# alessioGalatolo/GAN-2D-to-3D

Hardware: AMD Instinct MI355X
Metric: GAN2Shape step iters/sec, faces 128×128 b=8, 1/2/4/8 MI355X (higher is better)
Workload: dtype f32; 1 GPU; face128_n8; image_size=128, gan_size=128, n_proj_samples=8, mfma_operands=f32, prior=ellipsoid, step_mix=7:7:6 (step1:step2:step3, main.py:148 stage 0), images_per_rank=1

## Files before the change

### gan-2d-to-3d_amd/build.py

```python
import os
import subprocess
import sys

HERE = os.path.dirname(os.path.abspath(__file__))
CSRC = os.path.join(HERE, "csrc")
LIBDIR = os.path.join(HERE, "lib")
LIB = os.path.join(LIBDIR, "libg2s.so")
ARCH = "gfx950"

SOURCES = {
    "api.hip": [],
    "raster.hip": ["-ffp-contract=off"],
    "raster_rgb.hip": ["-ffp-contract=off"],
    "sweep.hip": ["-ffp-contract=off"],
    "face_light.hip": ["-ffp-contract=off"],
    "mapping.hip": ["-ffp-contract=off"],
    "fused_bias_act.hip": [],
    "upfirdn2d.hip": [],
    "modconv.hip": [],
    "modconv_f16.hip": [],
    "thinconv.hip": [],
    "winograd.hip": ["-fno-slp-vectorize"],
    "winograd4.hip": ["-fno-slp-vectorize"],
    "split_reduce.hip": [],
    "rowops.hip": [],
    "projector.hip": [],
    "synth_batch.hip": [],
    "lpips.hip": [],
    "pool.hip": [],
    "losses.hip": [],
    "geometry.hip": ["-ffp-contract=off"],
    "grid_sample.hip": ["-ffp-contract=off"],
    "priors.hip": ["-ffp-contract=off"],
    "metrics.hip": ["-ffp-contract=off"],
    "parsing.hip": [],
    "groupnorm.hip": [],
    "conv_wgrad.hip": [],
    "adam.hip": [],
    "probe.hip": [],
}
COMMON = ["--offload-arch=" + ARCH, "-O3", "-fPIC", "-std=c++17", "-Wall", "-Wno-unused-function",
          "-mllvm", "-instcombine-max-copied-from-constant-users=100000"]


def _newer(src, dst, deps):
    if not os.path.exists(dst):
        return True
    t = os.path.getmtime(dst)
    return any(os.path.getmtime(d) > t for d in [src] + deps)


def build(force=False, verbose=False):
    hipcc = os.environ.get("HIPCC", "/opt/rocm/bin/hipcc")
    os.makedirs(LIBDIR, exist_ok=True)
    headers = [os.path.join(CSRC, f) for f in os.listdir(CSRC) if f.endswith((".h", ".inc"))]
    headers.append(os.path.join(HERE, "..", "include", "g2s.h"))
    objs, jobs = [], []
    for name, extra in SOURCES.items():
        src = os.path.join(CSRC, name)
        if not os.path.exists(src):
            continue
# ... 26 lines not shown
```

### gan-2d-to-3d_amd/lib.py

```python
import ctypes as C
import os

import torch

_HERE = os.path.dirname(os.path.abspath(__file__))
LIB_PATH = os.path.join(_HERE, "lib", "libg2s.so")

G2S_F32, G2S_F16 = 0, 1
CONV_PLAIN, CONV_UP2, CONV_DOWN2 = 0, 1, 2

_lib = None

_p, _i, _f, _sz, _i64, _d = C.c_void_p, C.c_int, C.c_float, C.c_size_t, C.c_int64, C.c_double
SIGNATURES = {
    "g2s_abi_version": (_i, []),
    "g2s_last_error": (C.c_char_p, []),
    "g2s_clamp": (_i, [_p, _p, _p, _i64, _f, _f, _i, _p]),
    "g2s_avg_pyramid": (_i, [_p, _p, _i, _i64, _i, _i, _p]),
    "g2s_res_split_fwd": (_i, [_p, _p, _p, _i64, _i, _i, _p]),
    "g2s_res_split_bwd": (_i, [_p, _p, _p, _p, _i64, _i, _i, _p]),
    "g2s_depth_head_fwd": (_i, [_p, _p, _p, _i64, _i, _f, _f, _i, _f, _p]),
    "g2s_depth_head_bwd": (_i, [_p, _p, _p, _p, _p, _i64, _i, _f, _f, _i, _f, _i, _p]),
    "g2s_grid_sample_fwd": (_i, [_p, _p, _p, _i, _i, _i, _i, _i, _i, _i, _f, _f, _p]),
    "g2s_grid_sample_bwd_workspace_bytes": (_sz, [_i, _i, _i, _i]),
# ... 36 lines not shown
    "g2s_upfirdn2d_nba_ps": (_i, [_p, _p, _p] + [_i] * 12 + [_p, _p, _p, _f, _f, _p]),
    "g2s_synth_bwd_rows_ps": (_i, [_p] * 13 + [_i, _i, _i, _f, _f, _p]),
    "g2s_channel_sum": (_i, [_p, _p, _i, _i, _i, _p]),
    "g2s_noise_grad": (_i, [_p, _p, _p, _i, _i, _i, _p]),
    "g2s_noise_regularize_workspace_bytes": (_sz, [_p, _i, _i]),
    "g2s_noise_regularize": (_i, [_p, _p, _p, _i, _i, _p, _p, _sz, _p]),
    "g2s_noise_normalize_workspace_bytes": (_sz, [_p, _i, _i]),
    "g2s_noise_normalize": (_i, [_p, _p, _i, _i, _p, _sz, _p]),
    "g2s_demod_fwd_multi": (_i, [_p, _p, _p, _p, _p, _i, _i, _f, _p]),
    "g2s_demod_bwd_multi": (_i, [_p, _p, _p, _p, _p, _p, _p, _i, _i, _p]),
    "g2s_modconv_f16": (_i, [_p, _p, _p, _p, _p, _p, _i, _i, _i, _i, _i, _i, _i, _i, _i, _f, _f, _p]),
    "g2s_modconv_tune": (_i, [_i, _i]),
    "g2s_mfma_probe": (_i, [_p, _i, _i, _i, _p]),
    "g2s_mfma_lds_probe": (_i, [_p, _i, _i, _i, _i, _p]),
    "g2s_wino_weights_floats": (_sz, [_i, _i]),
    "g2s_wino4_weights_floats": (_sz, [_i, _i]),
    "g2s_wino4_weights": (_i, [_p, _p, _i, _i, _i, _p]),
    "g2s_wino4_supported": (_i, [_i] * 5),
    "g2s_conv3x3_wino4": (_i, [_p] * 8 + [_i] * 6 + [_f, _f, _i, _p, _i64, _p]),
    "g2s_wino_weights": (_i, [_p, _p, _i, _i, _i, _p]),
    "g2s_conv3x3_wino": (_i, [_p] * 8 + [_i] * 6 + [_f, _f, _i, _p, _i64, _p]),
    "g2s_conv2d": (_i, [_p, _p, _p, _p] + [_i] * 12 + [_i, _f, _f, _i, _i, _p]),
    "g2s_conv2d_wgrad": (_i, [_p, _p, _p] + [_i] * 10 + [_i, _i, _p]),
    "g2s_conv2d_bwd": (_i, [_p, _p, _p] + [_i] * 13 + [_p, _p, _p] + [_i] * 8 + [_p]),
    "g2s_adam_chunk": (_i64, []),
    "g2s_adam_step": (_i, [_p, _p, _p, _i, _i, _f, _f, _f, _f, _f, _p]),
    "g2s_rows_dot_scale": (_i, [_p, _p, _p, _p, _p, _p, _i, _i, _p]),
    "g2s_demod_fwd": (_i, [_p, _p, _p, _i, _i, _i, _f, _p]),
    "g2s_demod_bwd": (_i, [_p, _p, _p, _p, _p, _i, _i, _i, _p]),
    "g2s_demod_bwd_add": (_i, [_p, _p, _p, _p, _p, _p, _i, _i, _i, _p]),
    "g2s_lpips_layer_fwd": (_i, [_p, _p, _p, _p, _i, _i, _i, _p]),
    "g2s_lpips_layer_bwd": (_i, [_p, _p, _p, _p, _p, _i, _i, _i, _p]),
    "g2s_lpips_layer_bwd_ex": (_i, [_p, _p, _p, _p, _p, _i, _p, _i, _i, _i, _p]),
    "g2s_weighted_l1_fwd": (_i, [_p, _p, _p, _p, _i, _i, _i, _p]),
    "g2s_weighted_l1_bwd": (_i, [_p, _p, _p, _p, _p, _i, _i, _i, _p]),
    "g2s_weighted_l1_fwd2": (_i, [_p, _p, _p, _p, _i, _i, _i, _p]),
    "g2s_weighted_l1_bwd3": (_i, [_p] * 7 + [_f, _p, _p, _f, _f, _p, _i, _i, _i, _p]),
    "g2s_weighted_l1_bwd2": (_i, [_p, _p, _p, _p, _p, _p, _p, _i, _i, _i, _p]),
    "g2s_view_transform_fwd": (_i, [_p, _f, _f, _f, _p, _p, _i, _p]),
    "g2s_view_transform_bwd": (_i, [_p, _f, _f, _f, _p, _p, _p, _i, _p]),
    "g2s_warp_verts_fwd": (_i, [_p, _p, _p, _p, _f, _p, _i, _i, _p]),
    "g2s_warp_verts_bwd": (_i, [_p, _p, _p, _p, _f, _p, _p, _i, _i, _i, _p]),
    "g2s_inv_warp_grid_fwd": (_i, [_p, _p, _p, _p, _p, _f, _p, _i, _i, _i, _p]),
    "g2s_inv_warp_grid_bwd": (_i, [_p, _p, _p, _p, _p, _f, _p, _p, _p, _i, _i, _i, _i, _p]),
    "g2s_normal_fwd": (_i, [_p, _p, _p, _i, _i, _i, _p]),
    "g2s_normal_bwd": (_i, [_p, _p, _p, _p, _i, _i, _i, _p]),
    "g2s_shading_fwd": (_i, [_p, _p, _p, _p, _p, _i, _i, _i, _i, _p]),
    "g2s_shading_bwd": (_i, [_p, _p, _p, _p, _p, _p, _p, _p, _i, _i, _i, _i, _i, _p]),
    "g2s_smooth_loss_fwd": (_i, [_p, _p, _i, _i, _i, _i, _p]),
    "g2s_smooth_loss_bwd": (_i, [_p, _p, _p, _i, _i, _i, _p]),
    "g2s_groupnorm_workspace_floats": (_sz, [_i, _i, _i, _i]),
    "g2s_groupnorm_act_fwd": (_i, [_p, _p, _p, _p, _p, _p, _p, _i, _i, _i, _i, _f, _i, _f, _p]),
    "g2s_groupnorm_act_bwd": (_i, [_p, _p, _p, _p, _p, _p, _p, _p, _p, _p, _i, _i, _i, _i, _i, _f, _p]),
    "g2s_prior_map": (_i, [_p, _i, _i, _i, _d, _d, _p, _p]),
    "g2s_prior_smooth_workspace_bytes": (_sz, [_i, _i, _i, _i]),
    "g2s_prior_smooth": (_i, [_p, _i, _i, _i, _i, _d, _d, _p, _p, _sz, _p]),
    "g2s_prior_ellipsoid_workspace_bytes": (_sz, [_i]),
    "g2s_prior_ellipsoid": (_i, [_p, _i, _i, _d, _d, _d, _d, _p, _p, _sz, _p]),
    "g2s_conv_stem7": (_i, [_p, _p, _p, _p, _i, _i, _i, _i, _i, _p]),
    "g2s_maxpool3x3s2": (_i, [_p, _p, _i, _i, _i, _p]),
    "g2s_adaptive_avgpool": (_i, [_p, _p, _i, _i, _i, _i, _i, _p]),
    "g2s_resize_bilinear": (_i, [_p, _p, _i, _i, _i, _i, _i, _i, _p]),
    "g2s_gate_add_act": (_i, [_p, _p, _p, _p, _p, _i, _i, _i, _i, _i, _p]),
    "g2s_parse_head_workspace_bytes": (_sz, [_i]),
    "g2s_parse_head": (_i, [_p, _i, _i, _i, _i, _i, _i, _i, _i, C.c_uint32, _p, _p, _p, _p, _sz, _p]),
    "g2s_depth_metrics_workspace_bytes": (_sz, [_i, _i, _i]),
# ... 64 lines not shown
```

### gan-2d-to-3d_amd/lpips.py

```python
import torch
import torch.nn as nn
from torch.autograd import Function
from torch.autograd.function import once_differentiable

from . import lib as _lib
from . import zeropool

_VGG_SLICES = [
    [(0, 3, 64), (2, 64, 64)],
    [(5, 64, 128), (7, 128, 128)],
    [(10, 128, 256), (12, 256, 256), (14, 256, 256)],
    [(17, 256, 512), (19, 512, 512), (21, 512, 512)],
    [(24, 512, 512), (26, 512, 512), (28, 512, 512)],
]
_POOL_BEFORE = [None, 4, 9, 16, 23]


def normalize_tensor(in_feat, eps=1e-10):
    norm_factor = torch.sqrt(torch.sum(in_feat ** 2, dim=1, keepdim=True))
    return in_feat / (norm_factor + eps)


class _LpipsLayer(Function):

# ... 23 lines not shown

class _MaxPool2x2(Function):

    @staticmethod
    def forward(ctx, x):
        x = x.contiguous()
        B, C_, H, W = x.shape
        y = torch.empty((B, C_, H // 2, W // 2), dtype=torch.float32, device=x.device)
        _lib.check(_lib.load().g2s_maxpool2x2_fwd(_lib.ptr(x), _lib.ptr(y), B * C_, H, W, _lib.stream()))
        ctx.save_for_backward(x)
        return y

    @staticmethod
    def backward(ctx, gy):
        (x,) = ctx.saved_tensors
        B, C_, H, W = x.shape
        gx = torch.empty_like(x)
        _lib.check(_lib.load().g2s_maxpool2x2_bwd(_lib.ptr(x), _lib.ptr(gy.contiguous()), _lib.ptr(gx), B * C_, H, W,
                                                  _lib.stream()))
        return gx


def _pool_ok(mod):
    return (mod.kernel_size in (2, (2, 2)) and mod.stride in (2, (2, 2)) and mod.padding in (0, (0, 0))
            and not mod.ceil_mode and mod.dilation in (1, (1, 1)))


class _VggLpips(Function):

    SPLIT_FORWARD = False

    @staticmethod
    def forward(ctx, pred, target, net):
        from .modconv import conv_bias_act_raw
        N = pred.shape[0]
        sl = net.scaling_layer
        x = (torch.cat([pred, target], 0) - sl.shift) / sl.scale
        L = _lib.load()
        acc = zeropool.zeros(N, pred.device)
        saved = []
        for si in range(5):
            entry = {"pool_in": None, "convs": []}
            for mod in getattr(net.net, f"slice{si + 1}"):
                if isinstance(mod, nn.MaxPool2d):
                    entry["pool_in"] = x
                    B, C_, H, W = x.shape
                    y = torch.empty((B, C_, H // 2, W // 2), dtype=torch.float32, device=x.device)
                    _lib.check(L.g2s_maxpool2x2_fwd(_lib.ptr(x), _lib.ptr(y), B * C_, H, W, _lib.stream()))
                    x = y
                elif isinstance(mod, nn.Conv2d):
                    if _VggLpips.SPLIT_FORWARD:
                        x = torch.cat([conv_bias_act_raw(x[:N], mod.weight, mod.bias),
                                       conv_bias_act_raw(x[N:], mod.weight, mod.bias)], 0)
                    else:
                        x = conv_bias_act_raw(x, mod.weight, mod.bias)
                    entry["convs"].append((mod.weight, x))
            wv = getattr(net, f"lin{si}").model[-1].weight.reshape(-1).contiguous()
            C_, HW = x.shape[1], x.shape[2] * x.shape[3]
            _lib.check(L.g2s_lpips_layer_fwd(_lib.ptr(x[:N]), _lib.ptr(x[N:]), _lib.ptr(wv), _lib.ptr(acc),
                                             N, C_, HW, _lib.stream()))
            entry["lin"] = wv
            saved.append(entry)
        ctx.saved, ctx.N, ctx.scale = saved, N, sl.scale
        return acc.view(-1, 1, 1, 1)

    @staticmethod
    @once_differentiable
    def backward(ctx, gout):
        from .modconv import PLAIN, modconv_raw, relu_gate
        L = _lib.load()
        N = ctx.N
        gout = gout.contiguous().view(-1)
        g = None
        for si in range(4, -1, -1):
            e = ctx.saved[si]
            y = e["convs"][-1][1]
            C_, HW = y.shape[1], y.shape[2] * y.shape[3]
            gn = torch.empty((N,) + tuple(y.shape[1:]), dtype=torch.float32, device=y.device)
            _lib.check(L.g2s_lpips_layer_bwd_ex(_lib.ptr(y[:N]), _lib.ptr(y[N:]), _lib.ptr(e["lin"]), _lib.ptr(gout),
                                                _lib.ptr(g), 1, _lib.ptr(gn), N, C_, HW, _lib.stream()))
            g = gn
            convs = e["convs"]
            for ci in range(len(convs) - 1, -1, -1):
                w, yc = convs[ci]
                if ci != len(convs) - 1:
                    g = relu_gate(g, yc[:N])
                g = modconv_raw(g, w, None, None, PLAIN, 1)
            if e["pool_in"] is not None:
                xin = e["pool_in"]
                B2, C2, H, W = xin.shape
                gx = torch.empty((N, C2, H, W), dtype=torch.float32, device=xin.device)
                _lib.check(L.g2s_maxpool2x2_bwd(_lib.ptr(xin[:N]), _lib.ptr(g.contiguous()), _lib.ptr(gx), N * C2, H, W,
                                                _lib.stream()))
                g = gx
        return g / ctx.scale, None, None


def max_pool_2x2(mod, x):
    if (x.is_cuda and x.dtype == torch.float32 and x.dim() == 4 and x.shape[2] % 2 == 0 and x.shape[3] % 8 == 0
            and mod.kernel_size in (2, (2, 2)) and mod.stride in (2, (2, 2)) and mod.padding in (0, (0, 0))
            and not mod.ceil_mode and mod.dilation in (1, (1, 1))):
        return _MaxPool2x2.apply(x)
    return mod(x)


class VGG16Features(nn.Module):

    def __init__(self):
        super().__init__()
        for si, convs in enumerate(_VGG_SLICES):
            seq = nn.Sequential()
            if _POOL_BEFORE[si] is not None:
                seq.add_module(str(_POOL_BEFORE[si]), nn.MaxPool2d(kernel_size=2, stride=2))
            for idx, cin, cout in convs:
                seq.add_module(str(idx), nn.Conv2d(cin, cout, kernel_size=3, padding=1))
                seq.add_module(str(idx + 1), nn.ReLU(inplace=True))
            setattr(self, f"slice{si + 1}", seq)
        for p in self.parameters():
            p.requires_grad = False

    def forward(self, x):
        fused = x.is_cuda and x.dtype == torch.float32 and not any(p.requires_grad for p in self.parameters())
        outs = []
        for si in range(5):
            if fused:
                from .modconv import conv_bias_relu
                for mod in getattr(self, f"slice{si + 1}"):
                    if isinstance(mod, nn.Conv2d):
# ... 8 lines not shown

class ScalingLayer(nn.Module):
    def __init__(self):
        super().__init__()
        self.register_buffer('shift', torch.Tensor([-.030, -.088, -.188])[None, :, None, None])
        self.register_buffer('scale', torch.Tensor([.458, .448, .450])[None, :, None, None])

    def forward(self, inp):
        return (inp - self.shift) / self.scale


class NetLinLayer(nn.Module):
    def __init__(self, chn_in, chn_out=1, use_dropout=True):
        super().__init__()
        layers = [nn.Dropout()] if use_dropout else []
        layers += [nn.Conv2d(chn_in, chn_out, 1, stride=1, padding=0, bias=False)]
        self.model = nn.Sequential(*layers)


class PNetLin(nn.Module):

    ONE_NODE = True

    def __init__(self):
        super().__init__()
        self.scaling_layer = ScalingLayer()
        self.chns = [64, 128, 256, 512, 512]
        self.net = VGG16Features()
        for i, c in enumerate(self.chns):
            setattr(self, f"lin{i}", NetLinLayer(c))
        for p in self.parameters():
            p.requires_grad = False

    def features(self, x):
        return [normalize_tensor(f) for f in self.net(self.scaling_layer(x))]

    def forward(self, in0, in1):
        fused = in0.is_cuda and not in0.requires_grad and not any(
            getattr(self, f"lin{k}").model[-1].weight.requires_grad for k in range(5))
        if (fused and self.ONE_NODE and in0.dtype == torch.float32 and in0.shape == in1.shape
                and in0.shape[2] % 16 == 0 and in0.shape[3] % 64 == 0
                and not any(p.requires_grad for p in self.net.parameters())
                and all(_pool_ok(m) for s_ in range(1, 6) for m in getattr(self.net, f"slice{s_}")
                        if isinstance(m, nn.MaxPool2d))):
            return _VggLpips.apply(in1.contiguous(), in0.contiguous(), self)
        if not fused:
            f0, f1 = self.features(in0), self.features(in1)
            val = 0
            for k in range(5):
                diff = (f0[k] - f1[k]) ** 2
                val = val + getattr(self, f"lin{k}").model(diff).mean([2, 3], keepdim=True)
            return val
        with torch.no_grad():
            ft = self.net(self.scaling_layer(in0))
        fp = self.net(self.scaling_layer(in1))
        acc = torch.zeros(in1.shape[0], dtype=torch.float32, device=in1.device)
        for k in range(5):
            acc = _LpipsLayer.apply(fp[k], ft[k], getattr(self, f"lin{k}").model[-1].weight, acc)
        return acc.view(-1, 1, 1, 1)


class PerceptualLoss(nn.Module):

    def __init__(self, model='net-lin', net='vgg', use_gpu=True, gpu_ids=None,
                 lin_weights_path=None, vgg_weights_path=None):
        super().__init__()
        if model != 'net-lin' or net != 'vgg':
            raise NotImplementedError("only model='net-lin', net='vgg' (GAN2Shape/model.py:79)")
        self.net = PNetLin()
        self.pretrained = False
        if lin_weights_path is not None:
            self.load_lin_weights(lin_weights_path)
        if vgg_weights_path is not None:
            self.load_vgg_features(vgg_weights_path)
            self.pretrained = lin_weights_path is not None
        self.net.eval()

    def load_lin_weights(self, path):
        sd = path if isinstance(path, dict) else torch.load(path, map_location="cpu", weights_only=True)
        missing = self.net.load_state_dict(sd, strict=False)
        assert not [k for k in missing.unexpected_keys if k.startswith("lin")], missing

    def load_vgg_features(self, path):
        sd = path if isinstance(path, dict) else torch.load(path, map_location="cpu", weights_only=True)
        sd = {k.replace("features.", ""): v for k, v in sd.items() if "classifier" not in k}
        own = {}
        for si, convs in enumerate(_VGG_SLICES):
            for idx, _, _ in convs:
                for suffix in ("weight", "bias"):
                    own[f"slice{si + 1}.{idx}.{suffix}"] = sd[f"{idx}.{suffix}"]
        self.net.net.load_state_dict(own)

    def forward(self, pred, target, normalize=False):
        if normalize:
            target = 2 * target - 1
            pred = 2 * pred - 1
        return self.net(target, pred)
```

### gan-2d-to-3d_amd/model.py

```python
import datetime
import logging
import math
import os
from glob import glob

import torch
import torch.nn as nn
import torch.nn.functional as F
from torch.distributions.multivariate_normal import MultivariateNormal

from . import networks, utils, zeropool
from .op import grid_sample
from .losses import DiscriminatorLoss, PhotometricLoss, SmoothLoss
from .lpips import PerceptualLoss
from .renderer import Renderer
from .stylegan2 import Discriminator, Generator


_WSUM_CONST = {}


def weighted_total(terms):
    flat = [t.reshape(-1) for _, t in terms]
    per_elem = [tuple(float(v) for v in w) if isinstance(w, (tuple, list)) else (float(w) / f.numel(),) * f.numel()
                for (w, _), f in zip(terms, flat)]
    assert all(len(pe) == f.numel() for pe, f in zip(per_elem, flat))
    key = (tuple(per_elem), flat[0].device)
    wv = _WSUM_CONST.get(key)
    if wv is None:
        if flat[0].is_cuda and torch.cuda.is_current_stream_capturing():
            raise RuntimeError("weighted_total: first use of this weight vector under graph capture; run the step eagerly once")
        if len(_WSUM_CONST) > 64:
            _WSUM_CONST.clear()
        wv = _WSUM_CONST[key] = torch.tensor([v for pe in per_elem for v in pe], dtype=torch.float32).to(flat[0].device)
    return torch.dot(torch.cat(flat), wv)


class GAN2Shape(nn.Module):
    NETS = ['lighting', 'viewpoint', 'depth', 'albedo', 'offset_encoder']

    def __init__(self, config, debug=False, device="cuda"):
        super().__init__()
        self.device = torch.device(device)
        self.z_dim = config.get('z_dim')
        self.debug = debug
        self.generator = Generator(config.get('gan_size'), self.z_dim, 8,
                                   channel_multiplier=config.get('channel_multiplier'))
# ... 105 lines not shown
        if clamp_border:
            if self._depth_border is None or self._depth_border.shape[-2:] != (h, w):
                border = torch.zeros(1, h, w - 4, device=depth.device)
                self._depth_border = F.pad(border, (2, 2), mode='constant', value=1.02)
            depth = depth * (1 - self._depth_border) + self._depth_border * self.border_depth
        return depth

    def get_lighting_directions(self, lighting):
        lighting_a = lighting[:, :1] / 2 + 0.5
        lighting_b = lighting[:, 1:2] / 2 + 0.5
        lighting_d = torch.cat([lighting[:, 2:], lighting.new_ones(lighting.size(0), 1)], 1)
        lighting_d = lighting_d / ((lighting_d ** 2).sum(1, keepdim=True)) ** 0.5
        return lighting_a, lighting_b, lighting_d

    def get_shading(self, normal, lighting_a, lighting_b, lighting_d, albedo):
        diffuse_shading = (normal * lighting_d.view(-1, 1, 1, 3)).sum(3).clamp(min=0).unsqueeze(1)
        shading = lighting_a.view(-1, 1, 1, 1) + lighting_b.view(-1, 1, 1, 1) * diffuse_shading
        texture = (albedo / 2 + 0.5) * shading * 2 - 1
        return diffuse_shading, texture

    def _shade(self, normal, lighting, albedo):
        if lighting.is_cuda and self.renderer.fused:
            from .fused_geometry import shading
            diffuse_shading, texture = shading(normal, lighting, albedo)
            ab = lighting[:, :2] / 2 + 0.5
            return ab[:, :1], ab[:, 1:2], diffuse_shading, texture
        lighting_a, lighting_b, lighting_d = self.get_lighting_directions(lighting)
        diffuse_shading, texture = self.get_shading(normal, lighting_a, lighting_b, lighting_d, albedo)
        return lighting_a, lighting_b, diffuse_shading, texture

    @staticmethod
    def _head(x, n):
        return x if x.shape[0] == n else x[:n]

    def _no_grad_if(self, cond):
        return torch.no_grad() if cond else torch.enable_grad()

    def _fork(self, jobs):
        if len(jobs) < 2 or not self.parallel_nets or self.device.type != 'cuda':
            return [job() for job in jobs]
        main = torch.cuda.current_stream(self.device)
        while len(self._side_streams) < len(jobs) - 1:
            self._side_streams.append(torch.cuda.Stream(self.device))
        outs = [None] * len(jobs)
        for i, (job, side) in enumerate(zip(jobs[1:], self._side_streams), 1):
            side.wait_stream(main)
            with torch.cuda.stream(side):
                outs[i] = job()
        outs[0] = jobs[0]()
        for out, side in zip(outs[1:], self._side_streams):
            main.wait_stream(side)
            for t in (out if isinstance(out, (tuple, list)) else (out,)):
                t.record_stream(main)
        return outs

    def forward_step1(self, images, latents, collected, step1=True, eval=False, **kwargs):
        b = 1
        h, w = self.image_size, self.image_size
        if eval:
            zeropool.end()
        elif step1 and images.is_cuda:
            zeropool.begin(1, images.device)

        def frozen_if_step1(net, x):
            def job():
                with self._no_grad_if(step1):
                    return net(x)
            return job

        pre = kwargs.get('_nets')
        if pre is None and self.paired_nets:
            def vl_pair():
                with self._no_grad_if(step1):
                    return networks.forward_pair(self.viewpoint_net, self.lighting_net, images)
            (depth_raw, albedo), (view, lighting) = self._fork([
                lambda: networks.forward_pair(self.depth_net, self.albedo_net, images, train_a=not step1), vl_pair])
            if step1:
                depth_raw = depth_raw.detach()
        elif pre is None:
            depth_raw, albedo, view, lighting = self._fork([
                frozen_if_step1(self.depth_net, images), lambda: self.albedo_net(images),
                frozen_if_step1(self.viewpoint_net, images), frozen_if_step1(self.lighting_net, images)])
        else:
            depth_raw, albedo, view, lighting = pre
        depth = self.get_clamped_depth(depth_raw.squeeze(1), h, w)
        view = view + self.view_light_sampler.view_mean.unsqueeze(0)
        self._set_view(view)
        lighting = lighting + self.view_light_sampler.light_mean.unsqueeze(0)

        normal = self.renderer.get_normal_from_depth(depth)
        lighting_a, lighting_b, diffuse_shading, texture = self._shade(normal, lighting, albedo)

        recon_depth = self.renderer.warp_canon_depth(depth)
        grid_2d_from_canon = self.renderer.get_inv_warped_2d_grid(recon_depth)
        margin = (self.max_depth - self.min_depth) / 2
        recon_im_mask = (recon_depth < self.max_depth + margin).float().unsqueeze(1).detach()
        recon_im = grid_sample(texture, grid_2d_from_canon, -1, 1)
        if eval:
            return recon_im, recon_depth

        recon_b, mask_b = self._head(recon_im, b), self._head(recon_im_mask, b)
        loss_l1_im = self.photometric_loss(recon_b, images, mask=mask_b)
        perc_pair = (recon_b * mask_b, images * mask_b)
        smooth_terms = [(self.lam_smooth, self.smooth_loss(depth)), (self.lam_smooth, self.smooth_loss(diffuse_shading))]
        canon_mask = None if len(images) == 1 else [None] * len(images)
        collected = (normal, lighting_a, lighting_b, albedo, depth, canon_mask)
        if kwargs.get('_defer_perc'):
            return [(1.0, loss_l1_im)] + smooth_terms, collected, perc_pair
        loss_total = weighted_total([(1.0, loss_l1_im), (self.lam_perc, self.perceptual_loss(*perc_pair))] + smooth_terms)
        return loss_total, collected

    def _latent_centers(self):
        if self._centers is None:
            with torch.no_grad():
                zero = torch.zeros(1, self.z_dim, device=self.device)
                self._centers = (self.generator.style_forward(zero),
                                 self.generator.style_forward(zero, depth=8 - 2))
        return self._centers

    def forward_step2(self, image, latent, collected, n_proj_samples=8, **kwargs):
        F1_d = 2
        if image.is_cuda:
            zeropool.begin(2, image.device)
        *tensors, canon_mask = collected
        normal, light_a, light_b, albedo, depth = [t.detach() for t in tensors]

        with torch.no_grad():
            pseudo_im, mask = self.sample_pseudo_imgs(n_proj_samples, normal, light_a, light_b,
                                                      albedo, depth, canon_mask,
                                                      _draws=kwargs.get('_draws'))
            gan_im = None
            if self.relative_encoding:
                gan_im, _ = self.generator([latent], input_is_w=True,
                                           truncation_latent=self.mean_latent,
                                           truncation=self.truncation, randomize_noise=False)
                gan_im = utils.resize(gan_im.clamp(min=-1, max=1), [self.image_size, self.image_size])
            center_w, center_h = self._latent_centers()

        latent_projection = self.latent_projection(pseudo_im, gan_im, latent, center_w, center_h, F1_d)
        projected_image, offset = self.generator.invert(pseudo_im, latent_projection,
                                                        self.truncation, self.mean_latent)
        projected_image = utils.resize(projected_image, [self.image_size, self.image_size])
# ... 100 lines not shown
            if self.relative_encoding:
                gan_im, _ = self.generator([latent], input_is_w=True, truncation_latent=self.mean_latent,
                                           truncation=self.truncation, randomize_noise=False)
                gan_im = utils.resize(gan_im.clamp(min=-1, max=1), [self.image_size, self.image_size])
            center_w, center_h = self._latent_centers()
            offset, w = self.latent_projection(pseudo, gan_im, latent, center_w, center_h, F1_d)
            frames = []
            for i in range(0, V, gan_batch):
                j = slice(i, i + gan_batch)
                projected, _ = self.generator.invert(pseudo[j], (offset[j], w[j]), self.truncation, self.mean_latent)
                frames.append(utils.resize(projected, [self.image_size, self.image_size]))
        return dict(pseudo=pseudo, mask=mask, gan=torch.cat(frames, 0), w=w, view=d["view"], light=d["light"])

    def forward_step3(self, images, latents, collected, **kwargs):
        projected_samples, masks = collected
        if images.is_cuda:
            zeropool.begin(3, images.device)
        torch.randperm(len(projected_samples))
        projected_samples, masks = projected_samples.to(self.device), masks.to(self.device)

        b = len(projected_samples)
        both = torch.cat([images[:1], projected_samples], 0) if len(images) == 1 else None
        if both is not None:
            if self.paired_nets:
                (depth_raw, albedo1), (view_all, light_all) = self._fork([
                    lambda: networks.forward_pair(self.depth_net, self.albedo_net, images),
                    lambda: networks.forward_pair(self.viewpoint_net, self.lighting_net, both)])
            else:
                depth_raw, albedo1, view_all, light_all = self._fork([
                    lambda: self.depth_net(images), lambda: self.albedo_net(images),
                    lambda: self.viewpoint_net(both), lambda: self.lighting_net(both)])
            view1, view = view_all.split([1, b])
            light1, light = light_all.split([1, b])
            step1_loss, collected, perc1 = self.forward_step1(
                images, None, None, step1=False, _nets=(depth_raw, albedo1, view1, light1),
                _defer_perc=True)
        else:
            step1_loss, collected = self.forward_step1(images, None, None, step1=False)
            perc1 = None
            view, light = self.viewpoint_net(projected_samples), self.lighting_net(projected_samples)
        normal, _, _, albedo, depth, _ = collected

        view = view + self.view_light_sampler.view_mean.unsqueeze(0)
        self._set_view(view)
        light = light + self.view_light_sampler.light_mean.unsqueeze(0)
        _, _, diffuse_shading, texture = self._shade(normal, light, albedo)

        depth = depth.expand(b, self.image_size, self.image_size)
        recon_depth = self.renderer.warp_canon_depth(depth)
        grid_2d_from_canon = self.renderer.get_inv_warped_2d_grid(recon_depth)
        margin = (self.max_depth - self.min_depth) / 2
        recon_im_mask = (recon_depth < self.max_depth + margin).float().unsqueeze(1).detach() * masks
        recon_im = grid_sample(texture, grid_2d_from_canon, -1, 1)

        recon_b, mask_b = self._head(recon_im, b), self._head(recon_im_mask, b)
        loss_l1_im = self.photometric_loss(recon_b, projected_samples, mask=mask_b)
        pred, target = recon_b * mask_b, projected_samples * mask_b
        if perc1 is not None:
            perc = self.perceptual_loss(torch.cat([perc1[0], pred], 0), torch.cat([perc1[1], target], 0)).reshape(-1)
            terms = step1_loss + [(1.0, loss_l1_im), ((self.lam_perc,) + (self.lam_perc / b,) * b, perc)]
            return weighted_total(terms), None
        loss_perc_im = torch.mean(self.perceptual_loss(pred, target))
        return step1_loss + loss_l1_im + self.lam_perc * loss_perc_im, None

    def evaluate_results(self, image):
        with torch.no_grad():
            recon_im, recon_depth = self.forward_step1(image, None, None, eval=True)
            depth_raw = self.depth_net(image).squeeze(1)
            recon_depth = self.get_clamped_depth(depth_raw, self.image_size, self.image_size,
                                                 clamp_border=False)
        return recon_im, recon_depth

    def evaluate_results_masked(self, image, masking_model):
        recon_im, recon_depth = self.evaluate_results(image)
        return recon_im, masking_model.image_mask(image, recon_depth)

    def reinitialize_model(self):
        for name in GAN2Shape.NETS:
            for layer in getattr(self, f'{name}_net').modules():
                if hasattr(layer, 'reset_parameters'):
                    layer.reset_parameters()

    def save_checkpoint(self, img_idx, stage, total_it, category='car'):
        try:
            now = datetime.datetime.now().strftime("%Y_%m_%d_%H_%M")
            for net in GAN2Shape.NETS:
# ... 94 lines not shown
```

### include/g2s.h

```cpp
#ifndef G2S_H
#define G2S_H

#include <stddef.h>
#include <stdint.h>

#ifdef __cplusplus
extern "C" {
#endif

#define G2S_ABI_VERSION 1

#define G2S_OK 0
#define G2S_ERR_INVALID (-1)
#define G2S_ERR_LAUNCH (-2)
#define G2S_ERR_WORKSPACE (-3)

#define G2S_F32 0
#define G2S_F16 1

typedef void *g2s_stream_t;

int g2s_abi_version(void);
const char *g2s_last_error(void);

// ... 197 lines not shown
int g2s_demod_bwd_add(const float *wsq, const float *s, const float *demod, const float *gd, const float *gs_add,
                      float *gs, int B, int Cin, int Cout, g2s_stream_t stream);
int g2s_channel_sum(const float *g, float *out, int B, int C, int n, g2s_stream_t stream);
#define G2S_DEMOD_MAX_LAYERS 24
int g2s_demod_fwd_multi(const void *const *wsq, const void *const *s, const void *const *demod, const int *Cin,
                        const int *Cout, int layers, int B, float eps, g2s_stream_t stream);
int g2s_demod_bwd_multi(const void *const *wsq, const void *const *s, const void *const *demod, const void *const *gd,
                        const void *const *gs, const int *Cin, const int *Cout, int layers, int B, g2s_stream_t stream);
int g2s_synth_bwd_rows(const float *x, const float *g1, const float *s1, const float *g2, const float *s2,
                       const float *noise, const float *noise_w, const float *bias, const float *demod, float *out,
                       float *dot1, float *dot2, float *gdot, int rows, int channels, int n, float slope, float gain,
                       g2s_stream_t stream);
int g2s_synth_bwd_rows_ps(const float *x, const float *g1, const float *s1, const float *g2, const float *s2,
                          const float *noise, const float *noise_w, const float *bias, const float *demod, float *out,
                          float *dot1, float *dot2, float *gdot, int rows, int channels, int n, float slope, float gain,
                          g2s_stream_t stream);

#define G2S_NOISE_MAX_MAPS 32
int g2s_noise_grad(const float *gpre, const float *noise_w, float *gnoise, int B, int C, int n, g2s_stream_t stream);
size_t g2s_noise_regularize_workspace_bytes(const int *sides, int maps, int B);
int g2s_noise_regularize(const void *const *noise, const void *const *grad, const int *sides, int maps, int B,
                         float *loss, void *workspace, size_t workspace_bytes, g2s_stream_t stream);
size_t g2s_noise_normalize_workspace_bytes(const int *sides, int maps, int B);
int g2s_noise_normalize(const void *const *noise, const int *sides, int maps, int B, void *workspace,
                        size_t workspace_bytes, g2s_stream_t stream);

int g2s_lpips_layer_fwd(const float *f0, const float *f1, const float *w, float *out, int N, int C,
                        int HW, g2s_stream_t stream);
int g2s_lpips_layer_bwd(const float *f0, const float *f1, const float *w, const float *gout,
                        float *g0, int N, int C, int HW, g2s_stream_t stream);
int g2s_lpips_layer_bwd_ex(const float *f0, const float *f1, const float *w, const float *gout,
                           const float *g_in, int relu_gate, float *g0, int N, int C, int HW,
                           g2s_stream_t stream);

int g2s_weighted_l1_fwd(const float *x, const float *y, const float *w, float *num, int B, int C, int HW,
                        g2s_stream_t stream);
int g2s_weighted_l1_bwd(const float *x, const float *y, const float *w, const float *coef, float *gx, int B,
                        int C, int HW, g2s_stream_t stream);
int g2s_weighted_l1_fwd2(const float *x, const float *y, const float *w, float *numden, int B, int C, int HW,
                         g2s_stream_t stream);
int g2s_weighted_l1_bwd2(const float *x, const float *y, const float *w, const float *g, const float *den,
                         const float *gadd, float *gx, int B, int C, int HW, g2s_stream_t stream);
int g2s_weighted_l1_bwd3(const float *x, const float *y, const float *w, const float *g, const float *den,
                         const float *gadd, const float *gadd2, float add_scale, float *gx, const float *gate_ref,
                         float slope, float gain, float *gx_gate, int B, int C, int HW, g2s_stream_t stream);


int g2s_view_transform_fwd(const float *view, float rot_scale, float txy_scale, float tz_scale,
                           float *R, float *t, int B, g2s_stream_t stream);
int g2s_view_transform_bwd(const float *view, float rot_scale, float txy_scale, float tz_scale,
                           const float *gR, const float *gt, float *gview, int B, g2s_stream_t stream);
int g2s_warp_verts_fwd(const float *depth, const float *rays, const float *R, const float *t,
                       float rot_center_depth, float *verts, int B, int P, g2s_stream_t stream);
int g2s_warp_verts_bwd(const float *depth, const float *rays, const float *R, const float *gverts,
                       float rot_center_depth, float *gdepth, float *gRt, int B, int P, int acc_is_zero,
                       g2s_stream_t stream);
int g2s_inv_warp_grid_fwd(const float *depth, const float *rays, const float *R, const float *t,
                          const float *K, float rot_center_depth, float *grid, int B, int H, int W,
                          g2s_stream_t stream);
int g2s_inv_warp_grid_bwd(const float *depth, const float *rays, const float *R, const float *t,
                          const float *K, float rot_center_depth, const float *ggrid, float *gdepth,
                          float *gRt, int B, int H, int W, int acc_is_zero, g2s_stream_t stream);
int g2s_normal_fwd(const float *depth, const float *rays, float *normal, int B, int H, int W,
                   g2s_stream_t stream);
int g2s_normal_bwd(const float *depth, const float *rays, const float *gnormal, float *gdepth, int B,
                   int H, int W, g2s_stream_t stream);
// ... 51 lines not shown
```

Measured before the change: 206.6 iters/s.

## Fuse LPIPS input masking and normalization into one kernel writing a preassembled batch

Adds a kernel that computes the depth-threshold mask (optionally times the sample mask), applies it to the reconstruction and target images, and normalizes both directly into a preallocated LPIPS input buffer. The step-1 and step-3 paths add their rows into this shared buffer, which removes separate mask, multiply, concat and normalize ops. A matching backward kernel fuses the scale and mask gradient. The cost is more complex autograd plumbing with storage-aliased views, and new eligibility checks that fall back to the old path when they fail.

Result: slower. 204.5 iters/s (-1.0%).

```diff
diff --git a/gan-2d-to-3d_amd/build.py b/gan-2d-to-3d_amd/build.py
--- a/gan-2d-to-3d_amd/build.py
+++ b/gan-2d-to-3d_amd/build.py
@@ -27,6 +27,7 @@
     "projector.hip": [],
     "synth_batch.hip": [],
     "lpips.hip": [],
+    "tail.hip": ["-ffp-contract=off"],
     "pool.hip": [],
     "losses.hip": [],
     "geometry.hip": ["-ffp-contract=off"],
diff --git a/gan-2d-to-3d_amd/csrc/tail.hip b/gan-2d-to-3d_amd/csrc/tail.hip
--- /dev/null
+++ b/gan-2d-to-3d_amd/csrc/tail.hip
@@ -0,0 +1,109 @@
+#include "g2s_common.h"
+
+namespace g2s {
+
+struct LpipsFrontParams {
+    const float *recon, *target;
+    const float *depth;
+    const float *smask;
+    const float *shift, *scale;
+    float *xp, *xt;
+    float *mask;
+    float thr;
+    long N, HW;
+};
+
+template <int W> struct Lanes;
+template <> struct Lanes<4> { typedef float4 T; };
+template <> struct Lanes<1> { typedef float T; };
+
+template <int W, typename F>
+__device__ __forceinline__ typename Lanes<W>::T lanes_map(F f) {
+    if constexpr (W == 4) return make_float4(f(0), f(1), f(2), f(3));
+    else return f(0);
+}
+
+template <int W>
+__device__ __forceinline__ float lane_of(const typename Lanes<W>::T &v, int e) {
+    if constexpr (W == 4) return e == 0 ? v.x : e == 1 ? v.y : e == 2 ? v.z : v.w;
+    else return v;
+}
+
+template <int W>
+__global__ __launch_bounds__(256) void lpips_front_fwd(LpipsFrontParams p) {
+    typedef typename Lanes<W>::T V;
+    const long HWv = p.HW / W;
+    const long i = (long)blockIdx.x * 256 + threadIdx.x;
+    if (i >= p.N * HWv) return;
+    const long n = i / HWv, s = i - n * HWv;
+    const V d = reinterpret_cast<const V *>(p.depth)[i];
+    V m = lanes_map<W>([&](int e) { return lane_of<W>(d, e) < p.thr ? 1.0f : 0.0f; });
+    if (p.smask) {
+        const V sm = reinterpret_cast<const V *>(p.smask)[i];
+        m = lanes_map<W>([&](int e) { return lane_of<W>(m, e) * lane_of<W>(sm, e); });
+    }
+    reinterpret_cast<V *>(p.mask)[i] = m;
+#pragma unroll
+    for (int c = 0; c < 3; c++) {
+        const long j = (n * 3 + c) * HWv + s;
+        const float sh = p.shift[c], sc = p.scale[c];
+        const V r = reinterpret_cast<const V *>(p.recon)[j], t = reinterpret_cast<const V *>(p.target)[j];
+        reinterpret_cast<V *>(p.xp)[j] = lanes_map<W>([&](int e) { return (lane_of<W>(r, e) * lane_of<W>(m, e) - sh) / sc; });
+        reinterpret_cast<V *>(p.xt)[j] = lanes_map<W>([&](int e) { return (lane_of<W>(t, e) * lane_of<W>(m, e) - sh) / sc; });
+    }
+}
+
+template <int W>
+__global__ __launch_bounds__(256) void lpips_front_bwd(const float *__restrict__ g, const float *__restrict__ mask,
+                                                       const float *__restrict__ scale, float *__restrict__ gx,
+                                                       long N, long HW) {
+    typedef typename Lanes<W>::T V;
+    const long HWv = HW / W;
+    const long i = (long)blockIdx.x * 256 + threadIdx.x;
+    if (i >= N * HWv) return;
+    const long n = i / HWv, s = i - n * HWv;
+    const V m = reinterpret_cast<const V *>(mask)[i];
+#pragma unroll
+    for (int c = 0; c < 3; c++) {
+        const long j = (n * 3 + c) * HWv + s;
+        const float sc = scale[c];
+        const V a = reinterpret_cast<const V *>(g)[j];
+        reinterpret_cast<V *>(gx)[j] = lanes_map<W>([&](int e) { return (lane_of<W>(a, e) / sc) * lane_of<W>(m, e); });
+    }
+}
+
+static bool aligned16(std::initializer_list<const void *> ps) {
+    uintptr_t a = 0;
+    for (const void *q : ps) a |= (uintptr_t)q;
+    return (a & 15) == 0;
+}
+
+}
+
+using namespace g2s;
+
+extern "C" int g2s_lpips_front_fwd(const float *recon, const float *target, const float *depth, const float *smask,
+                                   const float *shift, const float *scale, float thr, float *xp, float *xt, float *mask,
+                                   int64_t N, int64_t HW, g2s_stream_t stream) {
+    G2S_REQUIRE(recon && target && depth && shift && scale && xp && xt && mask, "g2s_lpips_front_fwd: NULL pointer argument");
+    G2S_REQUIRE(N >= 1 && HW >= 1, "g2s_lpips_front_fwd: sizes must be positive");
+    G2S_REQUIRE(N * HW <= 0x7fffffffL * 64, "g2s_lpips_front_fwd: N * HW exceeds the grid");
+    LpipsFrontParams p{recon, target, depth, smask, shift, scale, xp, xt, mask, thr, (long)N, (long)HW};
+    const bool wide = HW % 4 == 0 && aligned16({recon, target, depth, smask, xp, xt, mask});
+    hipStream_t st = as_stream(stream);
+    if (wide) lpips_front_fwd<4><<<cdiv(N * HW / 4, 256), 256, 0, st>>>(p);
+    else lpips_front_fwd<1><<<cdiv(N * HW, 256), 256, 0, st>>>(p);
+    return check_launch("g2s_lpips_front_fwd");
+}
+
+extern "C" int g2s_lpips_front_bwd(const float *g, const float *mask, const float *scale, float *gx, int64_t N,
+                                   int64_t HW, g2s_stream_t stream) {
+    G2S_REQUIRE(g && mask && scale && gx, "g2s_lpips_front_bwd: NULL pointer argument");
+    G2S_REQUIRE(N >= 1 && HW >= 1, "g2s_lpips_front_bwd: sizes must be positive");
+    G2S_REQUIRE(N * HW <= 0x7fffffffL * 64, "g2s_lpips_front_bwd: N * HW exceeds the grid");
+    const bool wide = HW % 4 == 0 && aligned16({g, mask, gx});
+    hipStream_t st = as_stream(stream);
+    if (wide) lpips_front_bwd<4><<<cdiv(N * HW / 4, 256), 256, 0, st>>>(g, mask, scale, gx, (long)N, (long)HW);
+    else lpips_front_bwd<1><<<cdiv(N * HW, 256), 256, 0, st>>>(g, mask, scale, gx, (long)N, (long)HW);
+    return check_launch("g2s_lpips_front_bwd");
+}
diff --git a/gan-2d-to-3d_amd/lib.py b/gan-2d-to-3d_amd/lib.py
--- a/gan-2d-to-3d_amd/lib.py
+++ b/gan-2d-to-3d_amd/lib.py
@@ -92,6 +92,8 @@
     "g2s_lpips_layer_fwd": (_i, [_p, _p, _p, _p, _i, _i, _i, _p]),
     "g2s_lpips_layer_bwd": (_i, [_p, _p, _p, _p, _p, _i, _i, _i, _p]),
     "g2s_lpips_layer_bwd_ex": (_i, [_p, _p, _p, _p, _p, _i, _p, _i, _i, _i, _p]),
+    "g2s_lpips_front_fwd": (_i, [_p] * 6 + [_f, _p, _p, _p, _i64, _i64, _p]),
+    "g2s_lpips_front_bwd": (_i, [_p, _p, _p, _p, _i64, _i64, _p]),
     "g2s_weighted_l1_fwd": (_i, [_p, _p, _p, _p, _i, _i, _i, _p]),
     "g2s_weighted_l1_bwd": (_i, [_p, _p, _p, _p, _p, _i, _i, _i, _p]),
     "g2s_weighted_l1_fwd2": (_i, [_p, _p, _p, _p, _i, _i, _i, _p]),
diff --git a/gan-2d-to-3d_amd/lpips.py b/gan-2d-to-3d_amd/lpips.py
--- a/gan-2d-to-3d_amd/lpips.py
+++ b/gan-2d-to-3d_amd/lpips.py
@@ -79,12 +79,16 @@
 
     @staticmethod
     def forward(ctx, pred, target, net):
-        from .modconv import conv_bias_act_raw
-        N = pred.shape[0]
         sl = net.scaling_layer
         x = (torch.cat([pred, target], 0) - sl.shift) / sl.scale
+        ctx.scale = sl.scale
+        return _VggLpips.trunk_forward(ctx, x, pred.shape[0], net)
+
+    @staticmethod
+    def trunk_forward(ctx, x, N, net):
+        from .modconv import conv_bias_act_raw
         L = _lib.load()
-        acc = zeropool.zeros(N, pred.device)
+        acc = zeropool.zeros(N, x.device)
         saved = []
         for si in range(5):
             entry = {"pool_in": None, "convs": []}
@@ -108,12 +112,16 @@
                                              N, C_, HW, _lib.stream()))
             entry["lin"] = wv
             saved.append(entry)
-        ctx.saved, ctx.N, ctx.scale = saved, N, sl.scale
+        ctx.saved, ctx.N = saved, N
         return acc.view(-1, 1, 1, 1)
 
     @staticmethod
     @once_differentiable
     def backward(ctx, gout):
+        return _VggLpips.trunk_backward(ctx, gout) / ctx.scale, None, None
+
+    @staticmethod
+    def trunk_backward(ctx, gout):
         from .modconv import PLAIN, modconv_raw, relu_gate
         L = _lib.load()
         N = ctx.N
@@ -140,7 +148,74 @@
                 _lib.check(L.g2s_maxpool2x2_bwd(_lib.ptr(xin[:N]), _lib.ptr(g.contiguous()), _lib.ptr(gx), N * C2, H, W,
                                                 _lib.stream()))
                 g = gx
-        return g / ctx.scale, None, None
+        return g
+
+
+class _VggLpipsAssembled(Function):
+
+    @staticmethod
+    def forward(ctx, net, x, *parts):
+        ctx.rows = [p.shape[0] for p in parts]
+        return _VggLpips.trunk_forward(ctx, x, sum(ctx.rows), net)
+
+    @staticmethod
+    @once_differentiable
+    def backward(ctx, gout):
+        g = _VggLpips.trunk_backward(ctx, gout)
+        return (None, None) + tuple(g.split(ctx.rows))
+
+
+class _LpipsFront(Function):
+
+    @staticmethod
+    def forward(ctx, recon, target, depth, smask, thr, sl, x, row):
+        N, _, H, W = recon.shape
+        total = x.shape[0] // 2
+        recon, target, depth = recon.contiguous(), target.contiguous(), depth.contiguous()
+        smask = None if smask is None else smask.contiguous()
+        mask = torch.empty((N, 1, H, W), dtype=torch.float32, device=recon.device)
+        per = 3 * H * W
+
+        def rows(first):
+            return torch.empty(0, dtype=x.dtype, device=x.device).set_(
+                x.untyped_storage(), x.storage_offset() + first * per, (N, 3, H, W))
+        xp, xt = rows(row), rows(total + row)
+        scale = sl.scale.reshape(-1)
+        _lib.check(_lib.load().g2s_lpips_front_fwd(
+            _lib.ptr(recon), _lib.ptr(target), _lib.ptr(depth), _lib.ptr(smask), _lib.ptr(sl.shift.reshape(-1)),
+            _lib.ptr(scale), float(thr), _lib.ptr(xp), _lib.ptr(xt), _lib.ptr(mask), N, H * W, _lib.stream()))
+        ctx.save_for_backward(mask, scale)
+        ctx.mark_non_differentiable(mask)
+        return xp, mask
+
+    @staticmethod
+    @once_differentiable
+    def backward(ctx, g, _gmask):
+        mask, scale = ctx.saved_tensors
+        g = g.contiguous()
+        N, _, H, W = g.shape
+        gx = torch.empty_like(g)
+        _lib.check(_lib.load().g2s_lpips_front_bwd(_lib.ptr(g), _lib.ptr(mask), _lib.ptr(scale), _lib.ptr(gx), N, H * W,
+                                                   _lib.stream()))
+        return gx, None, None, None, None, None, None, None
+
+
+class LpipsInput:
+
+    def __init__(self, net, total, size, device):
+        self.net, self.total, self.row, self.parts = net, total, 0, []
+        self.x = torch.empty((2 * total, 3, size[0], size[1]), dtype=torch.float32, device=device)
+
+    def add(self, recon, target, depth, thr, smask=None):
+        assert self.row + recon.shape[0] <= self.total
+        xp, mask = _LpipsFront.apply(recon, target, depth, smask, thr, self.net.scaling_layer, self.x, self.row)
+        self.row += recon.shape[0]
+        self.parts.append(xp)
+        return mask
+
+    def loss(self):
+        assert self.row == self.total, "LpipsInput: rows missing"
+        return _VggLpipsAssembled.apply(self.net, self.x, *self.parts)
 
 
 def max_pool_2x2(mod, x):
@@ -215,17 +290,19 @@
         for p in self.parameters():
             p.requires_grad = False
 
+    def one_node_ok(self, h, w):
+        return (self.ONE_NODE and h % 16 == 0 and w % 64 == 0
+                and not any(p.requires_grad for p in self.parameters())
+                and all(_pool_ok(m) for s_ in range(1, 6) for m in getattr(self.net, f"slice{s_}")
+                        if isinstance(m, nn.MaxPool2d)))
+
     def features(self, x):
         return [normalize_tensor(f) for f in self.net(self.scaling_layer(x))]
 
     def forward(self, in0, in1):
         fused = in0.is_cuda and not in0.requires_grad and not any(
             getattr(self, f"lin{k}").model[-1].weight.requires_grad for k in range(5))
-        if (fused and self.ONE_NODE and in0.dtype == torch.float32 and in0.shape == in1.shape
-                and in0.shape[2] % 16 == 0 and in0.shape[3] % 64 == 0
-                and not any(p.requires_grad for p in self.net.parameters())
-                and all(_pool_ok(m) for s_ in range(1, 6) for m in getattr(self.net, f"slice{s_}")
-                        if isinstance(m, nn.MaxPool2d))):
+        if fused and in0.dtype == torch.float32 and in0.shape == in1.shape and self.one_node_ok(in0.shape[2], in0.shape[3]):
             return _VggLpips.apply(in1.contiguous(), in0.contiguous(), self)
         if not fused:
             f0, f1 = self.features(in0), self.features(in1)
@@ -274,6 +351,13 @@
                     own[f"slice{si + 1}.{idx}.{suffix}"] = sd[f"{idx}.{suffix}"]
         self.net.net.load_state_dict(own)
 
+    def assembled_input(self, total, recon, target):
+        if (recon.is_cuda and recon.dtype == torch.float32 and target.dtype == torch.float32 and recon.dim() == 4
+                and recon.shape[1] == 3 and recon.shape == target.shape and not target.requires_grad
+                and self.net.one_node_ok(recon.shape[2], recon.shape[3])):
+            return LpipsInput(self.net, total, recon.shape[2:], recon.device)
+        return None
+
     def forward(self, pred, target, normalize=False):
         if normalize:
             target = 2 * target - 1
diff --git a/gan-2d-to-3d_amd/model.py b/gan-2d-to-3d_amd/model.py
--- a/gan-2d-to-3d_amd/model.py
+++ b/gan-2d-to-3d_amd/model.py
@@ -12,7 +12,7 @@
 from . import networks, utils, zeropool
 from .op import grid_sample
 from .losses import DiscriminatorLoss, PhotometricLoss, SmoothLoss
-from .lpips import PerceptualLoss
+from .lpips import LpipsInput, PerceptualLoss
 from .renderer import Renderer
 from .stylegan2 import Discriminator, Generator
 
@@ -184,6 +184,10 @@
     @staticmethod
     def _head(x, n):
         return x if x.shape[0] == n else x[:n]
+
+    def _lpips_input(self, total, recon, target):
+        make = getattr(self.perceptual_loss, 'assembled_input', None)
+        return None if make is None else make(total, recon, target)
 
     def _no_grad_if(self, cond):
         return torch.no_grad() if cond else torch.enable_grad()
@@ -246,20 +250,28 @@
         recon_depth = self.renderer.warp_canon_depth(depth)
         grid_2d_from_canon = self.renderer.get_inv_warped_2d_grid(recon_depth)
         margin = (self.max_depth - self.min_depth) / 2
-        recon_im_mask = (recon_depth < self.max_depth + margin).float().unsqueeze(1).detach()
         recon_im = grid_sample(texture, grid_2d_from_canon, -1, 1)
         if eval:
             return recon_im, recon_depth
 
-        recon_b, mask_b = self._head(recon_im, b), self._head(recon_im_mask, b)
+        perc_pair = kwargs.get('_perc_input')
+        if perc_pair is None and recon_im.shape[0] == b and len(images) == b:
+            perc_pair = self._lpips_input(b, recon_im, images)
+        if perc_pair is not None:
+            recon_b = recon_im
+            mask_b = perc_pair.add(recon_im, images, recon_depth, self.max_depth + margin)
+        else:
+            recon_im_mask = (recon_depth < self.max_depth + margin).float().unsqueeze(1).detach()
+            recon_b, mask_b = self._head(recon_im, b), self._head(recon_im_mask, b)
+            perc_pair = (recon_b * mask_b, images * mask_b)
         loss_l1_im = self.photometric_loss(recon_b, images, mask=mask_b)
-        perc_pair = (recon_b * mask_b, images * mask_b)
         smooth_terms = [(self.lam_smooth, self.smooth_loss(depth)), (self.lam_smooth, self.smooth_loss(diffuse_shading))]
         canon_mask = None if len(images) == 1 else [None] * len(images)
         collected = (normal, lighting_a, lighting_b, albedo, depth, canon_mask)
         if kwargs.get('_defer_perc'):
             return [(1.0, loss_l1_im)] + smooth_terms, collected, perc_pair
-        loss_total = weighted_total([(1.0, loss_l1_im), (self.lam_perc, self.perceptual_loss(*perc_pair))] + smooth_terms)
+        perc = perc_pair.loss() if isinstance(perc_pair, LpipsInput) else self.perceptual_loss(*perc_pair)
+        loss_total = weighted_total([(1.0, loss_l1_im), (self.lam_perc, perc)] + smooth_terms)
         return loss_total, collected
 
     def _latent_centers(self):
@@ -426,9 +438,15 @@
                     lambda: self.viewpoint_net(both), lambda: self.lighting_net(both)])
             view1, view = view_all.split([1, b])
             light1, light = light_all.split([1, b])
+            perc_in = None
+            if masks.dim() == 4 and masks.shape[1] == 1 and masks.dtype == torch.float32 and not masks.requires_grad \
+                    and masks.shape[0] == b and masks.shape[2:] == projected_samples.shape[2:] \
+                    and projected_samples.shape[1:] == images.shape[1:] and not projected_samples.requires_grad \
+                    and projected_samples.dtype == torch.float32:
+                perc_in = self._lpips_input(1 + b, images, images)
             step1_loss, collected, perc1 = self.forward_step1(
                 images, None, None, step1=False, _nets=(depth_raw, albedo1, view1, light1),
-                _defer_perc=True)
+                _defer_perc=True, _perc_input=perc_in)
         else:
             step1_loss, collected = self.forward_step1(images, None, None, step1=False)
             perc1 = None
@@ -444,8 +462,13 @@
         recon_depth = self.renderer.warp_canon_depth(depth)
         grid_2d_from_canon = self.renderer.get_inv_warped_2d_grid(recon_depth)
         margin = (self.max_depth - self.min_depth) / 2
+        recon_im = grid_sample(texture, grid_2d_from_canon, -1, 1)
+        if isinstance(perc1, LpipsInput):
+            mask_b = perc1.add(recon_im, projected_samples, recon_depth, self.max_depth + margin, smask=masks)
+            loss_l1_im = self.photometric_loss(recon_im, projected_samples, mask=mask_b)
+            terms = step1_loss + [(1.0, loss_l1_im), ((self.lam_perc,) + (self.lam_perc / b,) * b, perc1.loss().reshape(-1))]
+            return weighted_total(terms), None
         recon_im_mask = (recon_depth < self.max_depth + margin).float().unsqueeze(1).detach() * masks
-        recon_im = grid_sample(texture, grid_2d_from_canon, -1, 1)
 
         recon_b, mask_b = self._head(recon_im, b), self._head(recon_im_mask, b)
         loss_l1_im = self.photometric_loss(recon_b, projected_samples, mask=mask_b)
diff --git a/include/g2s.h b/include/g2s.h
--- a/include/g2s.h
+++ b/include/g2s.h
@@ -253,6 +253,12 @@
 int g2s_lpips_layer_bwd_ex(const float *f0, const float *f1, const float *w, const float *gout,
                            const float *g_in, int relu_gate, float *g0, int N, int C, int HW,
                            g2s_stream_t stream);
+
+int g2s_lpips_front_fwd(const float *recon, const float *target, const float *depth, const float *smask,
+                        const float *shift, const float *scale, float thr, float *xp, float *xt, float *mask,
+                        int64_t N, int64_t HW, g2s_stream_t stream);
+int g2s_lpips_front_bwd(const float *g, const float *mask, const float *scale, float *gx, int64_t N, int64_t HW,
+                        g2s_stream_t stream);
 
 int g2s_weighted_l1_fwd(const float *x, const float *y, const float *w, float *num, int B, int C, int HW,
                         g2s_stream_t stream);
```
